# ax-le/nn-fac

Measured on NVIDIA B200. Metric: NMF outer iters/sec (HALS & MU beta=1) at 65536x8192 r=64, higher is better.
Workload: dtype f32

## Files before the change

### nn-fac_b200/csrc/tc_fused.cu

```cuda
#include "tc_plan.cuh"

#include <string.h>

namespace {
using namespace tcplan;

constexpr int NSP = 4;
constexpr int CW = 64 / NSP;
constexpr int NCHK = CW / 8;
constexpr int NWT = 4 * NSP;
constexpr int FUSED_THREADS = 128 + 32 * NWT;
static_assert(CW == 16, "the transform below moves 16 columns per tcgen05.ld / 8 words per tcgen05.st");
constexpr uint32_t X_BYTES = TILE_ROWS * BK * sizeof(bf16);
constexpr int MODE_RES = 0, MODE_MU = 1;
#ifndef FUSED_PREFETCH
#define FUSED_PREFETCH 0
#endif
#ifndef FUSED_PACKED
#define FUSED_PACKED 1
#endif
#ifndef FUSED_DEFER_COST
#define FUSED_DEFER_COST 1
#endif
constexpr int DRAIN = 2;

template <int RK>
struct Cfg {
  static constexpr int KR = RK / 64;
  static constexpr uint32_t FK_BYTES = (uint32_t)KR * 64 * BK * sizeof(bf16);
  static constexpr uint32_t STAGE_BYTES = 2 * X_BYTES + 2 * FK_BYTES;
  static constexpr int FSTAGES = RK == 64 ? 4 : 3;
  static constexpr int ND1 = RK == 64 ? 3 : 2;
  static constexpr uint32_t A1_BYTES = RK == 64 ? 2 * X_BYTES : 0;
  static constexpr int CWD = RK / NSP;
  static constexpr size_t SMEM = A1_BYTES + (size_t)FSTAGES * STAGE_BYTES + 512;
};

struct FusedParams {
  int r_pad, splits, stages_per_unit, num_units, drain, want_cost, tiles, split_major;
  int64_t ld_partial;
  float* partial;
  double* cost_part;
  const bf16 *a1h, *a1l;
  int64_t R;
  float* push[NNFAC_MAX_PEERS];
  int64_t push_chunk;
  int push_src;
};

__device__ __forceinline__ float rcp_approx(float x) {
  float y;
  asm("rcp.approx.ftz.f32 %0, %1;" : "=f"(y) : "f"(x));
  return y;
}
__device__ __forceinline__ float lg2_approx(float x) {
  float y;
  asm("lg2.approx.ftz.f32 %0, %1;" : "=f"(y) : "f"(x));
  return y;
}
__device__ __forceinline__ float bf_lo(uint32_t w) { return __uint_as_float(w << 16); }
__device__ __forceinline__ float bf_hi(uint32_t w) { return __uint_as_float(w & 0xffff0000u); }

template <int MODE, bool COST, bool XF32, int RK>
__global__ void __launch_bounds__(FUSED_THREADS, 1)
tc_fused_kernel(const __grid_constant__ CUtensorMap map_xh, const __grid_constant__ CUtensorMap map_xl,
                const __grid_constant__ CUtensorMap map_fkh, const __grid_constant__ CUtensorMap map_fkl,
                const __grid_constant__ CUtensorMap map_a1h, const __grid_constant__ CUtensorMap map_a1l,
                const FusedParams p) {
  using C = Cfg<RK>;
  static_assert(RK == 64 || (MODE == MODE_RES && !XF32), "rank 65..128: residual + cross-product pass only");
  constexpr int FSTAGES = C::FSTAGES, ND1 = C::ND1, CWD = C::CWD;
  constexpr uint32_t FK_BYTES = C::FK_BYTES, STAGE_BYTES = C::STAGE_BYTES, A1_BYTES = C::A1_BYTES;
  extern __shared__ __align__(1024) uint8_t smem[];
  uint8_t* a1 = smem;
  uint8_t* ring = smem + A1_BYTES;
  uint64_t* bars = reinterpret_cast<uint64_t*>(ring + (size_t)FSTAGES * STAGE_BYTES);
  uint64_t* full = bars;
  uint64_t* empty = bars + 4;
  uint64_t* a1_full = bars + 9;
  uint64_t* a1_empty = bars + 10;
  uint64_t* d1_full = bars + 11;
  uint64_t* d1_empty = bars + 14;
  uint64_t* d2_full = bars + 17;
  uint64_t* d2_empty = bars + 19;
  uint64_t* a1t_ready = bars + 21;
  uint64_t* a1t_free = bars + 22;
  uint64_t* q_ready = bars + 23;
  uint64_t* q_free = bars + 25;
  uint32_t* tmem_slot = reinterpret_cast<uint32_t*>(bars + 27);
  double* cost_sh = reinterpret_cast<double*>(bars + 28);

  const int warp = threadIdx.x >> 5, lane = threadIdx.x & 31;

  if (warp == 0 && lane == 0) {
    tc::prefetch_tmap(&map_xh); tc::prefetch_tmap(&map_xl);
    tc::prefetch_tmap(&map_fkh); tc::prefetch_tmap(&map_fkl);
    if (RK == 64) { tc::prefetch_tmap(&map_a1h); tc::prefetch_tmap(&map_a1l); }
  }
  if (warp == 1 && lane == 0) {
    for (int s = 0; s < FSTAGES; ++s) { tc::mbar_init(&full[s], 1); tc::mbar_init(&empty[s], NWT + 1); }
    tc::mbar_init(a1_full, 1); tc::mbar_init(a1_empty, NWT);
    tc::mbar_init(a1t_ready, NWT); tc::mbar_init(a1t_free, 1);
    for (int b = 0; b < 2; ++b) { tc::mbar_init(&q_ready[b], NWT); tc::mbar_init(&q_free[b], 1); }
    for (int b = 0; b < ND1; ++b) { tc::mbar_init(&d1_full[b], 1); tc::mbar_init(&d1_empty[b], NWT); }
    for (int b = 0; b < 2; ++b) { tc::mbar_init(&d2_full[b], 1); tc::mbar_init(&d2_empty[b], NWT); }
    tc::fence_barrier_init();
  }
  if (warp == 2) tc::tmem_alloc(tmem_slot, 512);
  tc::tcgen05_fence_before();
  __syncthreads();
  tc::tcgen05_fence_after();
  const uint32_t tmem_base = *tmem_slot;
  const uint32_t D1 = tmem_base, D2 = tmem_base + 64 * ND1, A1T = D2 + 2 * RK, QT = A1T + RK;
  const int S = p.stages_per_unit;

  if (warp == 0 && lane == 0) {
    int stage = 0; uint32_t phase = 0, a1_phase = 0;
    for (int u = blockIdx.x; u < p.num_units; u += gridDim.x) {
      const int tile = p.split_major ? u % p.tiles : u / p.splits, split = p.split_major ? u / p.tiles : u % p.splits;
      const int row0 = tile * TILE_ROWS, k0 = split * S * BK;
      if (RK == 64) {
        tc::mbar_wait(a1_empty, a1_phase ^ 1);
        a1_phase ^= 1;
        tc::mbar_arrive_expect_tx(a1_full, A1_BYTES);
        tc::tma_load_2d_hint(a1, &map_a1h, a1_full, 0, row0, tc::kEvictLast);
        tc::tma_load_2d_hint(a1 + X_BYTES, &map_a1l, a1_full, 0, row0, tc::kEvictLast);
      }
      for (int ks = 0; ks < S; ++ks) {
        tc::mbar_wait(&empty[stage], phase ^ 1);
        uint8_t* st = ring + (size_t)stage * STAGE_BYTES;
        tc::mbar_arrive_expect_tx(&full[stage], STAGE_BYTES);
        const int c = k0 + ks * BK;
        tc::tma_load_2d_hint(st, &map_xh, &full[stage], c, row0, tc::kEvictFirst);
        tc::tma_load_2d_hint(st + X_BYTES, XF32 ? &map_xh : &map_xl, &full[stage], XF32 ? c + 32 : c, row0, tc::kEvictFirst);
#pragma unroll
        for (int kr = 0; kr < C::KR; ++kr) {
          tc::tma_load_2d_hint(st + 2 * X_BYTES + kr * 8192, &map_fkh, &full[stage], kr * 64, c, tc::kEvictLast);
          tc::tma_load_2d_hint(st + 2 * X_BYTES + FK_BYTES + kr * 8192, &map_fkl, &full[stage], kr * 64, c, tc::kEvictLast);
        }
        if (++stage == FSTAGES) { stage = 0; phase ^= 1; }
      }
    }
  } else if (warp == 1) {
    const uint32_t idesc1 = tc::umma_idesc_bf16(TILE_ROWS, 64);
    const int ksteps = p.r_pad / UMMA_K;
    int st1 = 0; uint32_t ph1 = 0;
    int b1 = 0; uint32_t b1_phase = 0;
    uint32_t a1_phase = 0;
    for (int u = blockIdx.x; u < p.num_units; u += gridDim.x) {
      tc::mbar_wait(a1t_ready, a1_phase);
      a1_phase ^= 1;
      for (int i = 0; i < S; ++i) {
        tc::mbar_wait(&full[st1], ph1);
        tc::mbar_wait(&d1_empty[b1], b1_phase ^ 1);
        tc::tcgen05_fence_after();
        if (tc::elect_one()) {
          const uint32_t sb = tc::smem_u32(ring + (size_t)st1 * STAGE_BYTES);
          const uint64_t fkh = tc::umma_desc_k_sw128(sb + 2 * X_BYTES), fkl = tc::umma_desc_k_sw128(sb + 2 * X_BYTES + FK_BYTES);
          const uint32_t d = D1 + (uint32_t)b1 * 64;
#pragma unroll
          for (int k = 0; k < RK / UMMA_K; ++k) {
            if (k < ksteps) {
              const uint64_t bo = (uint64_t)((k >> 2) * (8192 >> 4) + (k & 3) * 2);
              tc::umma_bf16_ts(d, A1T + 8 * k, fkh + bo, idesc1, k != 0);
              tc::umma_bf16_ts(d, A1T + RK / 2 + 8 * k, fkh + bo, idesc1, true);
              tc::umma_bf16_ts(d, A1T + 8 * k, fkl + bo, idesc1, true);
            }
          }
          tc::umma_commit(&d1_full[b1]);
          if (i == S - 1) tc::umma_commit(a1t_free);
        }
        __syncwarp();
        if (++b1 == ND1) { b1 = 0; b1_phase ^= 1; }
        if (++st1 == FSTAGES) { st1 = 0; ph1 ^= 1; }
      }
    }
  } else if (warp == 3) {
    const uint32_t idesc2 = tc::umma_idesc_bf16(TILE_ROWS, p.r_pad) | (1u << 16);
    int qb = 0; uint32_t qb_phase = 0;
    int st2 = 0; uint32_t ph2 = 0;
    int b2 = 0; uint32_t b2_phase = 0;
    for (int u = blockIdx.x; u < p.num_units; u += gridDim.x) {
      for (int j = 0; j < S; ++j) {
        const bool chain_start = (j % DRAIN) == 0;
        const bool chain_end = ((j + 1) % DRAIN) == 0 || j == S - 1;
        tc::mbar_wait(&full[st2], ph2);
        if (MODE == MODE_MU) tc::mbar_wait(&q_ready[qb], qb_phase);
        if (chain_start) tc::mbar_wait(&d2_empty[b2], b2_phase ^ 1);
        tc::tcgen05_fence_after();
        if (tc::elect_one()) {
          const uint32_t sb = tc::smem_u32(ring + (size_t)st2 * STAGE_BYTES);
          const uint64_t xh = tc::umma_desc_k_sw128(sb), xl = tc::umma_desc_k_sw128(sb + X_BYTES);
          const uint64_t fnh = tc::umma_desc_mn_sw128(sb + 2 * X_BYTES);
          const uint64_t fnl = tc::umma_desc_mn_sw128(sb + 2 * X_BYTES + FK_BYTES);
          const uint32_t d = D2 + (uint32_t)b2 * RK;
#pragma unroll
          for (int k = 0; k < BK / UMMA_K; ++k) {
            const uint64_t ko = (uint64_t)(k * 2);
            const uint64_t kb = (uint64_t)(k * 128);
            if (MODE == MODE_MU) {
              const uint32_t qa = QT + (uint32_t)qb * 64 + 8 * k;
              tc::umma_bf16_ts(d, qa, fnh + kb, idesc2, !(chain_start && k == 0));
              tc::umma_bf16_ts(d, qa + 32, fnh + kb, idesc2, true);
              tc::umma_bf16_ts(d, qa, fnl + kb, idesc2, true);
            } else {
              tc::umma_bf16(d, xh + ko, fnh + kb, idesc2, !(chain_start && k == 0));
              tc::umma_bf16(d, xl + ko, fnh + kb, idesc2, true);
              tc::umma_bf16(d, xh + ko, fnl + kb, idesc2, true);
            }
          }
          tc::umma_commit(&empty[st2]);
          if (MODE == MODE_MU) tc::umma_commit(&q_free[qb]);
          if (chain_end) tc::umma_commit(&d2_full[b2]);
        }
        __syncwarp();
        if (MODE == MODE_MU) { if (++qb == 2) { qb = 0; qb_phase ^= 1; } }
        if (chain_end) { if (++b2 == 2) { b2 = 0; b2_phase ^= 1; } }
        if (++st2 == FSTAGES) { st2 = 0; ph2 ^= 1; }
      }
    }
  } else if (warp >= 4) {
    const int q = warp & 3, part = (warp - 4) >> 2;
    const int row = q * 32 + lane;
    const uint32_t lane_base = (uint32_t)(q * 32) << 16;
    int st = 0; uint32_t ph = 0;
    int b1 = 0; uint32_t b1_phase = 0;
    int b2 = 0; uint32_t b2_phase = 0;
    int qb = 0; uint32_t qb_phase = 0;
    uint32_t a1_phase = 0;
    double cost = 0.0, costk = 0.0;
    for (int u = blockIdx.x; u < p.num_units; u += gridDim.x) {
      const int tile = p.split_major ? u % p.tiles : u / p.splits, split = p.split_major ? u / p.tiles : u % p.splits;
      float sum[CWD];
#pragma unroll
      for (int j = 0; j < CWD; ++j) sum[j] = 0.f;
      if (RK == 64) {
        tc::mbar_wait(a1_full, a1_phase);
        tc::mbar_wait(a1t_free, a1_phase ^ 1);
        a1_phase ^= 1;
        tc::tcgen05_fence_after();
#pragma unroll
        for (int pl = 0; pl < 2; ++pl) {
          uint32_t w[4 * NCHK];
#pragma unroll
          for (int cc = 0; cc < NCHK; ++cc) {
            const int chunk = NCHK * part + cc;
            const uint4 v4 = *reinterpret_cast<const uint4*>(a1 + pl * X_BYTES + (uint32_t)row * 128u + (uint32_t)((chunk ^ (row & 7)) << 4));
            w[4 * cc] = v4.x; w[4 * cc + 1] = v4.y; w[4 * cc + 2] = v4.z; w[4 * cc + 3] = v4.w;
          }
          tc::tmem_st8(A1T + lane_base + 32 * pl + (CW / 2) * part, w);
        }
        tc::tmem_st_wait();
        tc::tcgen05_fence_before();
        __syncwarp();
        if (lane == 0) { tc::mbar_arrive(a1t_ready); tc::mbar_arrive(a1_empty); }
      } else {
        const int64_t grow = (int64_t)tile * TILE_ROWS + row;
        uint32_t w[2][16];
#pragma unroll
        for (int pl = 0; pl < 2; ++pl) {
          const uint4* src = reinterpret_cast<const uint4*>((pl ? p.a1l : p.a1h) + grow * RK + part * (RK / 4));
#pragma unroll
          for (int c = 0; c < 4; ++c) {
            const uint4 v4 = grow < p.R ? __ldg(src + c) : make_uint4(0u, 0u, 0u, 0u);
            w[pl][4 * c] = v4.x; w[pl][4 * c + 1] = v4.y; w[pl][4 * c + 2] = v4.z; w[pl][4 * c + 3] = v4.w;
          }
        }
        tc::mbar_wait(a1t_free, a1_phase ^ 1);
        a1_phase ^= 1;
        tc::tcgen05_fence_after();
        tc::tmem_st16(A1T + lane_base + (RK / 8) * part, w[0]);
        tc::tmem_st16(A1T + lane_base + RK / 2 + (RK / 8) * part, w[1]);
        tc::tmem_st_wait();
        tc::tcgen05_fence_before();
        __syncwarp();
        if (lane == 0) tc::mbar_arrive(a1t_ready);
      }
      auto drain_chain = [&]() {
        tc::mbar_wait(&d2_full[b2], b2_phase);
        tc::tcgen05_fence_after();
#pragma unroll
        for (int c0 = 0; c0 < CWD; c0 += 16) {
          if (CWD * part + c0 < p.r_pad) {
            uint32_t v[16];
            tc::tmem_ld16(D2 + (uint32_t)b2 * RK + lane_base + CWD * part + c0, v);
            tc::tmem_ld_wait();
#pragma unroll
            for (int j = 0; j < 16; ++j) sum[c0 + j] += __uint_as_float(v[j]);
          }
        }
        tc::tcgen05_fence_before();
        __syncwarp();
        if (lane == 0) tc::mbar_arrive(&d2_empty[b2]);
        if (++b2 == 2) { b2 = 0; b2_phase ^= 1; }
      };
      int drained = 0;
      float2 acc2 = make_float2(0.f, 0.f), acck2 = make_float2(0.f, 0.f);
      const float2 neg1 = make_float2(-1.f, -1.f), tiny2 = make_float2(1e-30f, 1e-30f);
      uint32_t kn[CW];
      int bf = b1; uint32_t bf_phase = b1_phase;
      auto fetch_d1 = [&]() {
        tc::mbar_wait(&d1_full[bf], bf_phase);
        tc::tcgen05_fence_after();
        tc::tmem_ld16(D1 + (uint32_t)bf * 64 + lane_base + CW * part, kn);
        if (++bf == ND1) { bf = 0; bf_phase ^= 1; }
      };
#if FUSED_PREFETCH
      fetch_d1();
#endif
      for (int i = 0; i < S; ++i) {
#if !FUSED_PREFETCH
        fetch_d1();
#endif
        tc::tmem_ld_wait16(kn);
        uint32_t kk[CW];
#pragma unroll
        for (int j = 0; j < CW; ++j) kk[j] = kn[j];
        tc::tcgen05_fence_before();
        __syncwarp();
        if (lane == 0) tc::mbar_arrive(&d1_empty[b1]);
        if (++b1 == ND1) { b1 = 0; b1_phase ^= 1; }
#if FUSED_PREFETCH
        if (i + 1 < S) fetch_d1();
#endif
        tc::mbar_wait(&full[st], ph);
        uint8_t* xh = ring + (size_t)st * STAGE_BYTES;
        uint8_t* xl = xh + X_BYTES;
        uint32_t qhw[4 * NCHK], qlw[4 * NCHK];
        constexpr bool DEFER = FUSED_DEFER_COST && FUSED_PACKED && MODE == MODE_MU && COST;
        float2 xs[DEFER ? 4 * NCHK : 1], qs[DEFER ? 4 * NCHK : 1];
#pragma unroll
        for (int cc = 0; cc < NCHK; ++cc) {
          float2 xv[4];
          if (XF32) {
            const uint8_t* xb = xh + (size_t)(part >> 1) * X_BYTES + (uint32_t)row * 128u;
#pragma unroll
            for (int h = 0; h < 2; ++h) {
              const int chunk = 4 * (part & 1) + 2 * cc + h;
              const float4 v4 = *reinterpret_cast<const float4*>(xb + ((chunk ^ (row & 7)) << 4));
              xv[2 * h] = make_float2(v4.x, v4.y); xv[2 * h + 1] = make_float2(v4.z, v4.w);
            }
          } else {
            const int chunk = NCHK * part + cc;
            const uint32_t off = (uint32_t)row * 128u + (uint32_t)((chunk ^ (row & 7)) << 4);
            const uint4 h4 = *reinterpret_cast<const uint4*>(xh + off);
            const uint4 l4 = *reinterpret_cast<const uint4*>(xl + off);
            const uint32_t hw[4] = {h4.x, h4.y, h4.z, h4.w}, lw[4] = {l4.x, l4.y, l4.z, l4.w};
#pragma unroll
            for (int w = 0; w < 4; ++w)
#if FUSED_PACKED
              xv[w] = __fadd2_rn(make_float2(bf_lo(hw[w]), bf_hi(hw[w])), make_float2(bf_lo(lw[w]), bf_hi(lw[w])));
#else
              xv[w] = make_float2(bf_lo(hw[w]) + bf_lo(lw[w]), bf_hi(hw[w]) + bf_hi(lw[w]));
#endif
          }
#if FUSED_PACKED
#pragma unroll
          for (int w = 0; w < 4; ++w) {
            const float2 x2 = xv[w];
            const float2 k2 = make_float2(__uint_as_float(kk[cc * 8 + 2 * w]), __uint_as_float(kk[cc * 8 + 2 * w + 1]));
            if (MODE == MODE_RES) {
              const float2 r2 = __ffma2_rn(k2, neg1, x2);
              acc2 = __ffma2_rn(r2, r2, acc2);
            } else {
              const float2 kt = __fadd2_rn(k2, tiny2);
              const float2 q2 = __fmul2_rn(x2, make_float2(rcp_approx(kt.x), rcp_approx(kt.y)));
              if (COST) {
                if (DEFER) {
                  xs[DEFER ? 4 * cc + w : 0] = x2; qs[DEFER ? 4 * cc + w : 0] = q2;
                } else {
                  const float2 qt = __fadd2_rn(q2, tiny2);
                  acc2 = __ffma2_rn(x2, make_float2(lg2_approx(qt.x), lg2_approx(qt.y)), acc2);
                }
                acck2 = __fadd2_rn(acck2, k2);
              }
              const __nv_bfloat162 hq = __floats2bfloat162_rn(q2.x, q2.y);
              const uint32_t hqw = *reinterpret_cast<const uint32_t*>(&hq);
              const float2 rem = __ffma2_rn(make_float2(bf_lo(hqw), bf_hi(hqw)), neg1, q2);
              const __nv_bfloat162 lq = __floats2bfloat162_rn(rem.x, rem.y);
              qhw[4 * cc + w] = hqw;
              qlw[4 * cc + w] = *reinterpret_cast<const uint32_t*>(&lq);
            }
          }
#else
#pragma unroll
          for (int w = 0; w < 4; ++w) {
            const float x0 = xv[w].x, x1 = xv[w].y;
            const float k0 = __uint_as_float(kk[cc * 8 + 2 * w]), k1 = __uint_as_float(kk[cc * 8 + 2 * w + 1]);
            if (MODE == MODE_RES) {
              const float r0 = x0 - k0, r1 = x1 - k1;
              acc2.x = fmaf(r0, r0, acc2.x);
              acc2.y = fmaf(r1, r1, acc2.y);
            } else {
              const float i0 = rcp_approx(fmaxf(k0, 1e-30f)), i1 = rcp_approx(fmaxf(k1, 1e-30f));
              const float q0 = x0 * i0, q1 = x1 * i1;
              if (COST) {
                acc2.x = fmaf(x0, lg2_approx(fmaxf(q0, 1e-30f)), acc2.x);
                acc2.y = fmaf(x1, lg2_approx(fmaxf(q1, 1e-30f)), acc2.y);
                acck2.x += k0; acck2.y += k1;
              }
              const __nv_bfloat162 hq = __floats2bfloat162_rn(q0, q1);
              const uint32_t hqw = *reinterpret_cast<const uint32_t*>(&hq);
              const __nv_bfloat162 lq = __floats2bfloat162_rn(q0 - bf_lo(hqw), q1 - bf_hi(hqw));
              qhw[4 * cc + w] = hqw;
              qlw[4 * cc + w] = *reinterpret_cast<const uint32_t*>(&lq);
            }
          }
#endif
        }
        auto flush_cost = [&]() {
          if (COST && ((i & 7) == 7 || i == S - 1)) {
            cost += (double)(acc2.x + acc2.y);
            acc2 = make_float2(0.f, 0.f);
            if (MODE == MODE_MU) { costk += (double)(acck2.x + acck2.y); acck2 = make_float2(0.f, 0.f); }
          }
        };
        if (!DEFER) flush_cost();
        __syncwarp();
        if (lane == 0) tc::mbar_arrive(&empty[st]);
        if (++st == FSTAGES) { st = 0; ph ^= 1; }
        if (MODE == MODE_MU) {
          tc::mbar_wait(&q_free[qb], qb_phase ^ 1);
          tc::tcgen05_fence_after();
          const uint32_t qa = QT + (uint32_t)qb * 64 + lane_base + (CW / 2) * part;
          tc::tmem_st8(qa, qhw);
          tc::tmem_st8(qa + 32, qlw);
          tc::tmem_st_wait();
          tc::tcgen05_fence_before();
          __syncwarp();
          if (lane == 0) tc::mbar_arrive(&q_ready[qb]);
          if (++qb == 2) { qb = 0; qb_phase ^= 1; }
          if (DEFER) {
#pragma unroll
            for (int e = 0; e < 4 * NCHK; ++e) {
              const float2 qt = __fadd2_rn(qs[DEFER ? e : 0], tiny2);
              acc2 = __ffma2_rn(xs[DEFER ? e : 0], make_float2(lg2_approx(qt.x), lg2_approx(qt.y)), acc2);
            }
            flush_cost();
          }
        }
        if (i >= 3 && (i & 1)) { drain_chain(); ++drained; }
      }
      for (; drained < (S + DRAIN - 1) / DRAIN; ++drained) drain_chain();
      if (p.push_chunk > 0) {
        const int64_t row0 = (int64_t)tile * TILE_ROWS;
        const int q = (int)(row0 / p.push_chunk);
        float* out = p.push[q] + (((int64_t)p.push_src * p.splits + split) * p.r_pad + CWD * part) * p.push_chunk + (row0 - q * p.push_chunk) + row;
#pragma unroll
        for (int j = 0; j < CWD; ++j)
          if (CWD * part + j < p.r_pad) out[(int64_t)j * p.push_chunk] = sum[j];
      } else {
        float* out = p.partial + ((int64_t)split * p.r_pad + CWD * part) * p.ld_partial + (int64_t)tile * TILE_ROWS + row;
#pragma unroll
        for (int j = 0; j < CWD; ++j)
          if (CWD * part + j < p.r_pad) out[(int64_t)j * p.ld_partial] = sum[j];
      }
    }
    if (COST) {
      cost = warp_sum(cost);
      if (MODE == MODE_MU) costk = warp_sum(costk);
      if (lane == 0) { cost_sh[warp - 4] = cost; cost_sh[NWT + warp - 4] = costk; }
      asm volatile("bar.sync 1, %0;" ::"n"(32 * NWT) : "memory");
      if (warp == 4 && lane == 0) {
        double t = 0.0, tk = 0.0;
        for (int w = 0; w < NWT; ++w) { t += cost_sh[w]; tk += cost_sh[NWT + w]; }
        p.cost_part[blockIdx.x] = t;
        p.cost_part[512 + blockIdx.x] = tk;
      }
    }
  }
  tc::tcgen05_fence_before();
  __syncthreads();
  if (warp == 2) tc::tmem_dealloc(tmem_base, 512);
}

struct PeerG {
  const float* p[NNFAC_MAX_PEERS];
  const unsigned long long* flags;
  int world;
  unsigned long long seq;
};

template <bool APPLY, int RK, bool PULL>
__global__ void __launch_bounds__(256) factor_finish_kernel(const float* __restrict__ partial, int splits, int r, int r_pad, int64_t R,
                                                            int64_t ldp, const float* __restrict__ F_in, int64_t ld_in,
                                                            int64_t in_chunk, int64_t in_slab, const PeerG G,
                                                            const float* __restrict__ den, float floor_value, float* __restrict__ F_out,
                                                            int64_t ld_out, bf16* __restrict__ fh, bf16* __restrict__ fl, int64_t ld_plane,
                                                            bf16* __restrict__ rowh, bf16* __restrict__ rowl) {
  __shared__ float tile[RK][33];
  const int tx = threadIdx.x & 31, ty = threadIdx.x >> 5;
  if (PULL && G.flags != nullptr) {
    if ((int)threadIdx.x < G.world) {
      const unsigned long long* f = G.flags + NNFAC_MAX_PEERS + threadIdx.x;
      unsigned long long v, spins = 0;
      do {
        asm volatile("ld.acquire.sys.global.u64 %0, [%1];" : "=l"(v) : "l"(f) : "memory");
        if (++spins > (1ull << 27)) __trap();
      } while (v < G.seq);
    }
    __syncthreads();
  }
  const int64_t c0 = (int64_t)blockIdx.x * 32, c = c0 + tx;
  const int64_t cin = in_chunk > 0 ? (c / in_chunk) * in_slab + (c % in_chunk) : c;
  float pulled[PULL ? RK / 8 : 1];
  if (PULL) {
    const float* src = c < R ? G.p[c / in_chunk] + (c % in_chunk) : nullptr;
#pragma unroll
    for (int i = 0; i < RK / 8; ++i) {
      const int k = ty + 8 * i;
      pulled[i] = (k < r && c < R) ? __ldcv(src + (int64_t)k * ld_in) : 0.f;
    }
  }
#pragma unroll
  for (int k = ty; k < RK; k += 8) {
    float f = 0.f;
    if (k < r && c < R) {
      f = PULL ? pulled[PULL ? (k - ty) / 8 : 0] : F_in[(int64_t)k * ld_in + cin];
      if (APPLY) {
        float num = 0.f;
        int sp = 0;
        for (; sp + 8 <= splits; sp += 8) {
          float t[8];
#pragma unroll
          for (int u = 0; u < 8; ++u) t[u] = partial[((int64_t)(sp + u) * r_pad + k) * ldp + c];
#pragma unroll
          for (int u = 0; u < 8; ++u) num += t[u];
        }
        for (; sp < splits; ++sp) num += partial[((int64_t)sp * r_pad + k) * ldp + c];
        const float v = f * (num / den[k]);
        f = v > floor_value ? v : floor_value;
        if (v != v) f = v;
      }
      if (F_out) F_out[(int64_t)k * ld_out + c] = f;
      bf16 h, l;
      tc::split_bf16(f, h, l);
      fh[(int64_t)k * ld_plane + c] = h;
      fl[(int64_t)k * ld_plane + c] = l;
    }
    tile[k][tx] = f;
  }
  if (rowh == nullptr) return;
  __syncthreads();
  for (int i = ty; i < 32; i += 8) {
    const int64_t cc = c0 + i;
    if (cc < R) {
#pragma unroll
      for (int h2 = 0; h2 < RK / 32; ++h2) {
        const int k = tx + 32 * h2;
        bf16 h, l;
        tc::split_bf16(tile[k][i], h, l);
        rowh[cc * RK + k] = h;
        rowl[cc * RK + k] = l;
      }
    }
  }
}

__global__ void sum_cost_parts_kernel(const double* part, int n, double* out) {
  if (threadIdx.x == 0) {
    double s = 0.0;
    for (int i = 0; i < n; ++i) s += part[i];
    out[0] = s;
  }
}

__global__ void kl_cost_finish_kernel(const double* part, int n, const double* sums, double* out) {
  if (threadIdx.x == 0) {
    double s = 0.0, sk = 0.0;
    for (int i = 0; i < n; ++i) { s += part[i]; sk += part[512 + i]; }
    constexpr double a0 = 6.05e-8, a1 = -4.0e-8;
    s = (1.0 - a1) * s - a0 * sums[0];
    out[0] = 0.6931471805599453 * s - sums[0] + sk;
  }
}

__global__ void __launch_bounds__(256) planes_to_f32_kernel(const bf16* __restrict__ hi, const bf16* __restrict__ lo, int64_t count,
                                                            float* __restrict__ out) {
  const int64_t stride = (int64_t)gridDim.x * blockDim.x * 2;
  for (int64_t i = ((int64_t)blockIdx.x * blockDim.x + threadIdx.x) * 2; i < count; i += stride) {
    const uint32_t h = *reinterpret_cast<const uint32_t*>(hi + i), l = *reinterpret_cast<const uint32_t*>(lo + i);
    *reinterpret_cast<float2*>(out + i) = make_float2(bf_lo(h) + bf_lo(l), bf_hi(h) + bf_hi(l));
  }
}

}

static int finish_factor(nnfac_nmf_plan* p, int which, bool apply, const float* F_in, int64_t ld_in, int64_t in_chunk, int64_t in_slab,
                         const float* den, float floor_value, float* F_out, int64_t ld_out, cudaStream_t st, const PeerG* pulled = nullptr) {
  const int64_t len = which == 0 ? p->m : p->n;
  Side* cs = &p->side[which == 0 ? 1 : 0];
  Side* ps = &p->side[which];
  const unsigned grid = (unsigned)ceil_div64(len, 32);
  bf16* rh = p->fused_ok ? p->rowp_h[which] : nullptr;
  bf16* rl = p->fused_ok ? p->rowp_l[which] : nullptr;
  PeerG none;
  memset(&none, 0, sizeof(none));
#define NNFAC_FINISH(RKV)                                                                                                          \
  do {                                                                                                                             \
    if (pulled)                                                                                                                    \
      factor_finish_kernel<false, RKV, true><<<grid, 256, 0, st>>>(nullptr, 0, p->r, p->r_pad, len, 0, nullptr, ld_in, in_chunk,  \
          in_slab, *pulled, nullptr, 0.f, F_out, ld_out, cs->fh, cs->fl, cs->ld, rh, rl);                                          \
    else if (apply)                                                                                                                \
      factor_finish_kernel<true, RKV, false><<<grid, 256, 0, st>>>(p->partial, ps->cp.splits, p->r, p->r_pad, len,                \
          ps->cp.ld_partial, F_in, ld_in, in_chunk, in_slab, none, den, floor_value, F_out, ld_out, cs->fh, cs->fl, cs->ld, rh,    \
          rl);                                                                                                                     \
    else                                                                                                                           \
      factor_finish_kernel<false, RKV, false><<<grid, 256, 0, st>>>(nullptr, 0, p->r, p->r_pad, len, 0, F_in, ld_in, in_chunk,    \
          in_slab, none, nullptr, 0.f, F_out, ld_out, cs->fh, cs->fl, cs->ld, rh, rl);                                             \
  } while (0)
  if (p->rk == 64) NNFAC_FINISH(64); else NNFAC_FINISH(128);
#undef NNFAC_FINISH
  NNFAC_LAUNCH_CHECK(p->ctx);
  return NNFAC_OK;
}

extern "C" {

int nnfac_nmf_plan_f32_bytes(const nnfac_nmf_plan* p, size_t* bytes) {
  NNFAC_ARG(p && bytes, "nnfac_nmf_plan_f32_bytes: NULL argument");
  size_t tot = 0;
  for (int i = 0; i < 2; ++i) tot += (((size_t)p->side[i].R * p->side[i].ld * sizeof(float)) + 255) & ~(size_t)255;
  *bytes = tot;
  return NNFAC_OK;
}

int nnfac_nmf_plan_enable_f32(nnfac_nmf_plan* p, void* workspace, size_t workspace_bytes, void* stream) {
  NNFAC_ARG(p && workspace && (((uintptr_t)workspace) & 255) == 0, "nnfac_nmf_plan_enable_f32: bad argument");
  size_t need = 0;
  nnfac_nmf_plan_f32_bytes(p, &need);
  NNFAC_ARG(workspace_bytes >= need, "nnfac_nmf_plan_enable_f32: workspace of %zu bytes needed, got %zu", need, workspace_bytes);
  NNFAC_ARG(p->sides == 3, "nnfac_nmf_plan_enable_f32: needs a two-sided plan");
  if (!p->fused_ok || p->rk != 64) { nnfac_set_error("nnfac_nmf_plan_enable_f32: rank %d > 64 is not covered by the beta = 1 fused pass", p->r); return NNFAC_ERR_UNSUPPORTED; }
  cudaStream_t st = (cudaStream_t)stream;
  uint8_t* base = (uint8_t*)workspace;
  for (int i = 0; i < 2; ++i) {
    Side* s = &p->side[i];
    p->xf[i] = (float*)base;
    const int64_t count = s->R * s->ld;
    base += (((size_t)count * sizeof(float)) + 255) & ~(size_t)255;
    planes_to_f32_kernel<<<p->ctx->sm_count * 16, 256, 0, st>>>(s->xh, s->xl, count, p->xf[i]);
    NNFAC_LAUNCH_CHECK(p->ctx);
    const int rc = make_map_f32(&p->map_xf[i], p->xf[i], s->R, s->C, s->ld);
    if (rc) return rc;
  }
  p->xf_ready = 1;
  return NNFAC_OK;
}

int nnfac_nmf_plan_set_factor(nnfac_nmf_plan* p, int which, const float* Ft, int64_t ld, void* stream) {
  NNFAC_ARG(p && Ft && (which == 0 || which == 1), "nnfac_nmf_plan_set_factor: bad argument");
  NNFAC_ARG(!p->base, "nnfac_nmf_plan_set_factor: not available on a view plan");
  const int64_t len = which == 0 ? p->m : p->n;
  NNFAC_ARG(ld >= len, "nnfac_nmf_plan_set_factor: leading dimension too small");
  return finish_factor(p, which, false, Ft, ld, 0, 0, nullptr, 0.f, nullptr, 0, (cudaStream_t)stream);
}

int nnfac_nmf_plan_set_factor_gathered(nnfac_nmf_plan* p, int which, const float* G, int64_t chunk, float* Ft_out, int64_t ld_out,
                                       void* stream) {
  NNFAC_ARG(p && G && Ft_out && chunk > 0 && (which == 0 || which == 1), "nnfac_nmf_plan_set_factor_gathered: bad argument");
  const int64_t len = which == 0 ? p->m : p->n;
  NNFAC_ARG(ld_out >= len, "nnfac_nmf_plan_set_factor_gathered: leading dimension too small");
  return finish_factor(p, which, false, G, chunk, chunk, (int64_t)p->r * chunk, nullptr, 0.f, Ft_out, ld_out, (cudaStream_t)stream);
}

const float* nnfac_xchg_peer_send(const nnfac_xchg* x, int q);
int nnfac_xchg_world(const nnfac_xchg* x);
void nnfac_xchg_wait_args(const nnfac_xchg* x, int phase, const unsigned long long** flags, int* world, unsigned long long* seq);
int nnfac_nmf_plan_set_factor_pulled(nnfac_nmf_plan* p, int which, const nnfac_xchg* x, int64_t chunk, int64_t pitch, float* Ft_out,
                                     int64_t ld_out, void* stream) {
  NNFAC_ARG(p && x && Ft_out && chunk > 0 && pitch >= chunk && (which == 0 || which == 1), "nnfac_nmf_plan_set_factor_pulled: bad argument");
  NNFAC_ARG(!p->base, "nnfac_nmf_plan_set_factor_pulled: not available on a view plan");
  const int64_t len = which == 0 ? p->m : p->n;
  const int world = nnfac_xchg_world(x);
  NNFAC_ARG(ld_out >= len && (int64_t)world * chunk >= len, "nnfac_nmf_plan_set_factor_pulled: %d slices of %lld columns do not cover %lld",
            world, (long long)chunk, (long long)len);
  PeerG g;
  for (int q = 0; q < NNFAC_MAX_PEERS; ++q) g.p[q] = nnfac_xchg_peer_send(x, q);
  nnfac_xchg_wait_args(x, 1, &g.flags, &g.world, &g.seq);
  return finish_factor(p, which, false, nullptr, pitch, chunk, 0, nullptr, 0.f, Ft_out, ld_out, (cudaStream_t)stream, &g);
}

int nnfac_nmf_plan_hals_solve(nnfac_nmf_plan* p, int which, const float* UtM, int64_t ld_utm, const float* UtU, int64_t ld_utu,
                              const float* F_in, int64_t ld_in, float* F_out, int64_t ld_out, int maxiter, double delta,
                              double sparsity, double* result, void* stream) {
  NNFAC_ARG(p && UtU && F_in && F_out && result && (which == 0 || which == 1), "nnfac_nmf_plan_hals_solve: bad argument");
  NNFAC_ARG(!p->base, "nnfac_nmf_plan_hals_solve: not available on a view plan");
  const int64_t len = which == 0 ? p->m : p->n;
  NNFAC_ARG((!UtM || ld_utm >= len) && ld_in >= len && ld_out >= len && ld_utu >= p->r, "nnfac_nmf_plan_hals_solve: leading dimension too small");
  int nsplit = 1;
  int64_t split_stride = 0;
  if (!UtM) {
    const CrossParams& cp = p->side[which].cp;
    UtM = p->partial; ld_utm = cp.ld_partial; nsplit = cp.splits; split_stride = (int64_t)p->r_pad * cp.ld_partial;
  }
  Side* cs = &p->side[which == 0 ? 1 : 0];
  nnfac_sweep_planes pl;
  pl.fh = cs->fh; pl.fl = cs->fl; pl.ld_plane = cs->ld; pl.r_pad = p->r_pad;
  pl.rowh = p->fused_ok ? p->rowp_h[which] : nullptr;
  pl.rowl = p->fused_ok ? p->rowp_l[which] : nullptr;
  pl.row_pitch = p->rk;
  return nnfac_tc_sweep_run(p->ctx, UtM, ld_utm, UtU, ld_utu, F_in, ld_in, F_out, ld_out, p->r, len, maxiter, delta, sparsity,
                            result, &pl, (cudaStream_t)stream, nsplit, split_stride);
}

void* nnfac_xchg_peer_stage(const nnfac_xchg* x, int q);
int nnfac_xchg_rank(const nnfac_xchg* x);
int64_t nnfac_xchg_stage_floats(const nnfac_xchg* x);
int nnfac_nmf_plan_set_push(nnfac_nmf_plan* p, const nnfac_xchg* x, int64_t inbox_off, int64_t chunk, int* slabs, int64_t* slab_stride) {
  NNFAC_ARG(p, "nnfac_nmf_plan_set_push: NULL plan");
  if (!x) { p->push_chunk = 0; return NNFAC_OK; }
  NNFAC_ARG(!p->base && p->fused_ok, "nnfac_nmf_plan_set_push: needs a plan with the fused pass");
  const int world = nnfac_xchg_world(x);
  const int splits = p->side[0].cp.splits;
  NNFAC_ARG(chunk > 0 && chunk % TILE_ROWS == 0 && (int64_t)world * chunk >= p->m && inbox_off >= 0,
            "nnfac_nmf_plan_set_push: %d slices of %lld rows (multiple of 128) must cover %lld", world, (long long)chunk, (long long)p->m);
  NNFAC_ARG(inbox_off + (int64_t)world * splits * p->r_pad * chunk <= nnfac_xchg_stage_floats(x),
            "nnfac_nmf_plan_set_push: the stage buffer is too small for %d x %d slabs of %d x %lld", world, splits, p->r_pad, (long long)chunk);
  for (int q = 0; q < world; ++q) p->push[q] = (float*)nnfac_xchg_peer_stage(x, q) + inbox_off;
  p->push_chunk = chunk; p->push_src = nnfac_xchg_rank(x); p->push_world = world;
  if (slabs) *slabs = world * splits;
  if (slab_stride) *slab_stride = (int64_t)p->r_pad * chunk;
  return NNFAC_OK;
}

int nnfac_reduce_slabs_f32(nnfac_ctx* ctx, const float* slabs, int64_t ld, int nslabs, int r, int r_pad, int64_t n, float* out,
                           int64_t ld_out, void* stream) {
  NNFAC_ARG(ctx && slabs && out && nslabs >= 1 && r >= 1 && r_pad >= r && n >= 1 && ld >= n && ld_out >= n, "nnfac_reduce_slabs_f32: bad argument");
  nnfac_reduce_partials(slabs, nslabs, r, r_pad, n, ld, out, ld_out, ctx->sm_count, (cudaStream_t)stream);
  NNFAC_LAUNCH_CHECK(ctx);
  return NNFAC_OK;
}

int nnfac_nmf_plan_reduce(nnfac_nmf_plan* p, int side, float* out, int64_t ld_out, void* stream) {
  NNFAC_ARG(p && out && (side == 0 || side == 1), "nnfac_nmf_plan_reduce: bad argument");
  Side* s = &p->side[side];
  NNFAC_ARG(ld_out >= s->R, "nnfac_nmf_plan_reduce: leading dimension too small");
  nnfac_reduce_partials(p->partial, s->cp.splits, p->r, p->r_pad, s->R, s->cp.ld_partial, out, ld_out, p->ctx->sm_count, (cudaStream_t)stream);
  NNFAC_LAUNCH_CHECK(p->ctx);
  return NNFAC_OK;
}

int nnfac_nmf_plan_reduce_chunked(nnfac_nmf_plan* p, int side, float* out, int64_t chunk, int slabs, const float* tail, int64_t ld_tail,
                                  int tail_cols, void* stream) {
  NNFAC_ARG(p && out && (side == 0 || side == 1) && chunk > 0 && slabs > 0 && tail_cols >= 0 && (tail || tail_cols == 0),
            "nnfac_nmf_plan_reduce_chunked: bad argument");
  Side* s = &p->side[side];
  NNFAC_ARG((int64_t)slabs * chunk >= s->R, "nnfac_nmf_plan_reduce_chunked: %d slabs of %lld columns do not cover %lld", slabs,
            (long long)chunk, (long long)s->R);
  nnfac_reduce_partials_chunked(p->partial, s->cp.splits, p->r, p->r_pad, s->R, s->cp.ld_partial, out, chunk, slabs, tail, ld_tail,
                                tail_cols, p->ctx->sm_count, (cudaStream_t)stream);
  NNFAC_LAUNCH_CHECK(p->ctx);
  return NNFAC_OK;
}

int nnfac_nmf_plan_mu_finish(nnfac_nmf_plan* p, int which, const float* F_in, int64_t ld_in, const float* den, double floor_value,
                             float* F_out, int64_t ld_out, void* stream) {
  NNFAC_ARG(p && F_in && den && F_out && (which == 0 || which == 1), "nnfac_nmf_plan_mu_finish: bad argument");
  const int64_t len = which == 0 ? p->m : p->n;
  NNFAC_ARG(ld_in >= len && ld_out >= len, "nnfac_nmf_plan_mu_finish: leading dimension too small");
  if (!p->fused_ok) { nnfac_set_error("nnfac_nmf_plan_mu_finish: rank %d > 128 is not covered by the fused pass", p->r); return NNFAC_ERR_UNSUPPORTED; }
  return finish_factor(p, which, true, F_in, ld_in, 0, 0, den, (float)floor_value, F_out, ld_out, (cudaStream_t)stream);
}

int nnfac_nmf_plan_fused(nnfac_nmf_plan* p, int side, int mode, int want_cost, float* out, int64_t ld_out, double* cost_out,
                         void* stream) {
  NNFAC_ARG(p && (side == 0 || side == 1) && (mode == 0 || mode == 1), "nnfac_nmf_plan_fused: bad argument");
  NNFAC_ARG((p->sides >> side) & 1, "nnfac_nmf_plan_fused: this plan keeps no planes of side %d", side);
  if (!p->fused_ok) { nnfac_set_error("nnfac_nmf_plan_fused: not covered by the fused pass (rank %d > 128, or a view plan)", p->r); return NNFAC_ERR_UNSUPPORTED; }
  if (mode == 1 && p->rk != 64) { nnfac_set_error("nnfac_nmf_plan_fused: the beta = 1 pass covers rank <= 64 (rank %d)", p->r); return NNFAC_ERR_UNSUPPORTED; }
  Side* s = &p->side[side];
  NNFAC_ARG(!out || ld_out >= s->R, "nnfac_nmf_plan_fused: leading dimension too small");
  cudaStream_t st = (cudaStream_t)stream;
  FusedParams fp;
  fp.r_pad = p->r_pad; fp.splits = s->cp.splits; fp.stages_per_unit = s->cp.stages_per_unit; fp.num_units = s->cp.num_units;
  fp.drain = DRAIN; fp.want_cost = (mode == 0 || want_cost) ? 1 : 0;
  fp.tiles = s->cp.tiles; fp.split_major = s->cp.split_major;
  fp.ld_partial = s->cp.ld_partial; fp.partial = p->partial; fp.cost_part = p->cost_part;
  fp.a1h = p->rowp_h[side]; fp.a1l = p->rowp_l[side]; fp.R = s->R;
  fp.push_chunk = 0; fp.push_src = 0;
  for (int q = 0; q < NNFAC_MAX_PEERS; ++q) fp.push[q] = nullptr;
  if (side == 0 && !out && p->push_chunk > 0) {
    fp.push_chunk = p->push_chunk; fp.push_src = p->push_src;
    for (int q = 0; q < p->push_world; ++q) fp.push[q] = p->push[q];
  }
  const int other = 1 - side;
#define NNFAC_LAUNCH_FUSED(M, C, XF, RKV, MAPH, MAPL)                                                                             \
  do {                                                                                                                        \
    const size_t smem = Cfg<RKV>::SMEM;                                                                                       \
    NNFAC_CUDA(cudaFuncSetAttribute(tc_fused_kernel<M, C, XF, RKV>, cudaFuncAttributeMaxDynamicSharedMemorySize, (int)smem)); \
    tc_fused_kernel<M, C, XF, RKV><<<s->grid, FUSED_THREADS, smem, st>>>(MAPH, MAPL, p->map_row_b_h[other],                  \
        p->map_row_b_l[other], p->map_row_a_h[side], p->map_row_a_l[side], fp);                                               \
  } while (0)
  if (mode == 0 && p->rk == 128) NNFAC_LAUNCH_FUSED(MODE_RES, true, false, 128, s->map_xh, s->map_xl);
  else if (mode == 0) NNFAC_LAUNCH_FUSED(MODE_RES, true, false, 64, s->map_xh, s->map_xl);
  else if (p->xf_ready) {
    if (fp.want_cost) NNFAC_LAUNCH_FUSED(MODE_MU, true, true, 64, p->map_xf[side], p->map_xf[side]);
    else NNFAC_LAUNCH_FUSED(MODE_MU, false, true, 64, p->map_xf[side], p->map_xf[side]);
  } else {
    if (fp.want_cost) NNFAC_LAUNCH_FUSED(MODE_MU, true, false, 64, s->map_xh, s->map_xl);
    else NNFAC_LAUNCH_FUSED(MODE_MU, false, false, 64, s->map_xh, s->map_xl);
  }
#undef NNFAC_LAUNCH_FUSED
  NNFAC_LAUNCH_CHECK(p->ctx);
  if (out) {
    nnfac_reduce_partials(p->partial, fp.splits, p->r, p->r_pad, s->R, fp.ld_partial, out, ld_out, p->ctx->sm_count, st);
    NNFAC_LAUNCH_CHECK(p->ctx);
  }
  if (cost_out && fp.want_cost) {
    if (mode == 0)
      sum_cost_parts_kernel<<<1, 32, 0, st>>>(p->cost_part, s->grid, cost_out);
    else
      kl_cost_finish_kernel<<<1, 32, 0, st>>>(p->cost_part, s->grid, p->sums, cost_out);
    NNFAC_LAUNCH_CHECK(p->ctx);
  }
  return NNFAC_OK;
}

}
```

Measured before the change: 776.5.

## Split fused kernel smem ring into separate X and factor rings with independent producers

Splits the single shared-memory stage ring (X tile plus factor slices) into two rings with their own full/empty barriers and a second TMA producer warp, so X and factor loads progress independently. The factor ring is released by the MMA warps via commits, while the X ring is released by the transform warps. In residual mode the X ring is released early, right after the values are read into registers. This lets factor stages be recycled without waiting for the slower elementwise consumers. The cost is more barriers, extra registers for X values held across the loop, and configurable ring depths that must fit in shared memory.

```diff
diff --git a/nn-fac_b200/csrc/tc_fused.cu b/nn-fac_b200/csrc/tc_fused.cu
--- a/nn-fac_b200/csrc/tc_fused.cu
+++ b/nn-fac_b200/csrc/tc_fused.cu
@@ -19,21 +19,43 @@
 #ifndef FUSED_PACKED
 #define FUSED_PACKED 1
 #endif
+#ifndef FUSED_X_FIRST
+#define FUSED_X_FIRST 0
+#endif
+#ifndef FUSED_MU_LATE_X
+#define FUSED_MU_LATE_X 1
+#endif
 #ifndef FUSED_DEFER_COST
 #define FUSED_DEFER_COST 1
 #endif
 constexpr int DRAIN = 2;
+#ifndef FUSED_XST64
+#define FUSED_XST64 4
+#endif
+#ifndef FUSED_SST64
+#define FUSED_SST64 4
+#endif
+#ifndef FUSED_XST128
+#define FUSED_XST128 3
+#endif
+#ifndef FUSED_SST128
+#define FUSED_SST128 3
+#endif
 
 template <int RK>
 struct Cfg {
   static constexpr int KR = RK / 64;
   static constexpr uint32_t FK_BYTES = (uint32_t)KR * 64 * BK * sizeof(bf16);
-  static constexpr uint32_t STAGE_BYTES = 2 * X_BYTES + 2 * FK_BYTES;
-  static constexpr int FSTAGES = RK == 64 ? 4 : 3;
+  static constexpr uint32_t XS_BYTES = 2 * X_BYTES;
+  static constexpr uint32_t SS_BYTES = 2 * FK_BYTES;
+  static constexpr int XST = RK == 64 ? FUSED_XST64 : FUSED_XST128;
+  static constexpr int SST = RK == 64 ? FUSED_SST64 : FUSED_SST128;
   static constexpr int ND1 = RK == 64 ? 3 : 2;
   static constexpr uint32_t A1_BYTES = RK == 64 ? 2 * X_BYTES : 0;
   static constexpr int CWD = RK / NSP;
-  static constexpr size_t SMEM = A1_BYTES + (size_t)FSTAGES * STAGE_BYTES + 512;
+  static constexpr int NBAR = 2 * XST + 2 * SST + 2 * ND1 + 10;
+  static constexpr size_t SMEM = A1_BYTES + (size_t)XST * XS_BYTES + (size_t)SST * SS_BYTES + 8 * (NBAR + 1 + 2 * NWT);
+  static_assert(SMEM <= 227 * 1024, "ring depths exceed the shared memory of a block");
 };
 
 struct FusedParams {
@@ -69,26 +91,30 @@
                 const FusedParams p) {
   using C = Cfg<RK>;
   static_assert(RK == 64 || (MODE == MODE_RES && !XF32), "rank 65..128: residual + cross-product pass only");
-  constexpr int FSTAGES = C::FSTAGES, ND1 = C::ND1, CWD = C::CWD;
-  constexpr uint32_t FK_BYTES = C::FK_BYTES, STAGE_BYTES = C::STAGE_BYTES, A1_BYTES = C::A1_BYTES;
+  constexpr int XST = C::XST, SST = C::SST, ND1 = C::ND1, CWD = C::CWD;
+  constexpr uint32_t FK_BYTES = C::FK_BYTES, XS_BYTES = C::XS_BYTES, SS_BYTES = C::SS_BYTES, A1_BYTES = C::A1_BYTES;
   extern __shared__ __align__(1024) uint8_t smem[];
   uint8_t* a1 = smem;
-  uint8_t* ring = smem + A1_BYTES;
-  uint64_t* bars = reinterpret_cast<uint64_t*>(ring + (size_t)FSTAGES * STAGE_BYTES);
-  uint64_t* full = bars;
-  uint64_t* empty = bars + 4;
-  uint64_t* a1_full = bars + 9;
-  uint64_t* a1_empty = bars + 10;
-  uint64_t* d1_full = bars + 11;
-  uint64_t* d1_empty = bars + 14;
-  uint64_t* d2_full = bars + 17;
-  uint64_t* d2_empty = bars + 19;
-  uint64_t* a1t_ready = bars + 21;
-  uint64_t* a1t_free = bars + 22;
-  uint64_t* q_ready = bars + 23;
-  uint64_t* q_free = bars + 25;
-  uint32_t* tmem_slot = reinterpret_cast<uint32_t*>(bars + 27);
-  double* cost_sh = reinterpret_cast<double*>(bars + 28);
+  uint8_t* xring = smem + A1_BYTES;
+  uint8_t* sring = xring + (size_t)XST * XS_BYTES;
+  uint64_t* bars = reinterpret_cast<uint64_t*>(sring + (size_t)SST * SS_BYTES);
+  uint64_t* x_full = bars;
+  uint64_t* x_empty = x_full + XST;
+  uint64_t* s_full = x_empty + XST;
+  uint64_t* s_empty = s_full + SST;
+  uint64_t* a1_full = s_empty + SST;
+  uint64_t* a1_empty = a1_full + 1;
+  uint64_t* d1_full = a1_empty + 1;
+  uint64_t* d1_empty = d1_full + ND1;
+  uint64_t* d2_full = d1_empty + ND1;
+  uint64_t* d2_empty = d2_full + 2;
+  uint64_t* a1t_ready = d2_empty + 2;
+  uint64_t* a1t_free = a1t_ready + 1;
+  uint64_t* q_ready = a1t_free + 1;
+  uint64_t* q_free = q_ready + 2;
+  static_assert(2 * XST + 2 * SST + 2 * ND1 + 10 == C::NBAR, "barrier block");
+  uint32_t* tmem_slot = reinterpret_cast<uint32_t*>(bars + C::NBAR);
+  double* cost_sh = reinterpret_cast<double*>(bars + C::NBAR + 1);
 
   const int warp = threadIdx.x >> 5, lane = threadIdx.x & 31;
 
@@ -98,7 +124,8 @@
     if (RK == 64) { tc::prefetch_tmap(&map_a1h); tc::prefetch_tmap(&map_a1l); }
   }
   if (warp == 1 && lane == 0) {
-    for (int s = 0; s < FSTAGES; ++s) { tc::mbar_init(&full[s], 1); tc::mbar_init(&empty[s], NWT + 1); }
+    for (int s = 0; s < XST; ++s) { tc::mbar_init(&x_full[s], 1); tc::mbar_init(&x_empty[s], MODE == MODE_MU ? NWT : NWT + 1); }
+    for (int s = 0; s < SST; ++s) { tc::mbar_init(&s_full[s], 1); tc::mbar_init(&s_empty[s], 2); }
     tc::mbar_init(a1_full, 1); tc::mbar_init(a1_empty, NWT);
     tc::mbar_init(a1t_ready, NWT); tc::mbar_init(a1t_free, 1);
     for (int b = 0; b < 2; ++b) { tc::mbar_init(&q_ready[b], NWT); tc::mbar_init(&q_free[b], 1); }
@@ -115,6 +142,21 @@
   const int S = p.stages_per_unit;
 
   if (warp == 0 && lane == 0) {
+    int stage = 0; uint32_t phase = 0;
+    for (int u = blockIdx.x; u < p.num_units; u += gridDim.x) {
+      const int tile = p.split_major ? u % p.tiles : u / p.splits, split = p.split_major ? u / p.tiles : u % p.splits;
+      const int row0 = tile * TILE_ROWS, k0 = split * S * BK;
+      for (int ks = 0; ks < S; ++ks) {
+        tc::mbar_wait(&x_empty[stage], phase ^ 1);
+        uint8_t* st = xring + (size_t)stage * XS_BYTES;
+        tc::mbar_arrive_expect_tx(&x_full[stage], XS_BYTES);
+        const int c = k0 + ks * BK;
+        tc::tma_load_2d_hint(st, &map_xh, &x_full[stage], c, row0, tc::kEvictFirst);
+        tc::tma_load_2d_hint(st + X_BYTES, XF32 ? &map_xh : &map_xl, &x_full[stage], XF32 ? c + 32 : c, row0, tc::kEvictFirst);
+        if (++stage == XST) { stage = 0; phase ^= 1; }
+      }
+    }
+  } else if (warp == 2 && lane == 0) {
     int stage = 0; uint32_t phase = 0, a1_phase = 0;
     for (int u = blockIdx.x; u < p.num_units; u += gridDim.x) {
       const int tile = p.split_major ? u % p.tiles : u / p.splits, split = p.split_major ? u / p.tiles : u % p.splits;
@@ -127,18 +169,16 @@
         tc::tma_load_2d_hint(a1 + X_BYTES, &map_a1l, a1_full, 0, row0, tc::kEvictLast);
       }
       for (int ks = 0; ks < S; ++ks) {
-        tc::mbar_wait(&empty[stage], phase ^ 1);
-        uint8_t* st = ring + (size_t)stage * STAGE_BYTES;
-        tc::mbar_arrive_expect_tx(&full[stage], STAGE_BYTES);
+        tc::mbar_wait(&s_empty[stage], phase ^ 1);
+        uint8_t* st = sring + (size_t)stage * SS_BYTES;
+        tc::mbar_arrive_expect_tx(&s_full[stage], SS_BYTES);
         const int c = k0 + ks * BK;
-        tc::tma_load_2d_hint(st, &map_xh, &full[stage], c, row0, tc::kEvictFirst);
-        tc::tma_load_2d_hint(st + X_BYTES, XF32 ? &map_xh : &map_xl, &full[stage], XF32 ? c + 32 : c, row0, tc::kEvictFirst);
 #pragma unroll
         for (int kr = 0; kr < C::KR; ++kr) {
-          tc::tma_load_2d_hint(st + 2 * X_BYTES + kr * 8192, &map_fkh, &full[stage], kr * 64, c, tc::kEvictLast);
-          tc::tma_load_2d_hint(st + 2 * X_BYTES + FK_BYTES + kr * 8192, &map_fkl, &full[stage], kr * 64, c, tc::kEvictLast);
-        }
-        if (++stage == FSTAGES) { stage = 0; phase ^= 1; }
+          tc::tma_load_2d_hint(st + kr * 8192, &map_fkh, &s_full[stage], kr * 64, c, tc::kEvictLast);
+          tc::tma_load_2d_hint(st + FK_BYTES + kr * 8192, &map_fkl, &s_full[stage], kr * 64, c, tc::kEvictLast);
+        }
+        if (++stage == SST) { stage = 0; phase ^= 1; }
       }
     }
   } else if (warp == 1) {
@@ -151,12 +191,12 @@
       tc::mbar_wait(a1t_ready, a1_phase);
       a1_phase ^= 1;
       for (int i = 0; i < S; ++i) {
-        tc::mbar_wait(&full[st1], ph1);
+        tc::mbar_wait(&s_full[st1], ph1);
         tc::mbar_wait(&d1_empty[b1], b1_phase ^ 1);
         tc::tcgen05_fence_after();
         if (tc::elect_one()) {
-          const uint32_t sb = tc::smem_u32(ring + (size_t)st1 * STAGE_BYTES);
-          const uint64_t fkh = tc::umma_desc_k_sw128(sb + 2 * X_BYTES), fkl = tc::umma_desc_k_sw128(sb + 2 * X_BYTES + FK_BYTES);
+          const uint32_t sb = tc::smem_u32(sring + (size_t)st1 * SS_BYTES);
+          const uint64_t fkh = tc::umma_desc_k_sw128(sb), fkl = tc::umma_desc_k_sw128(sb + FK_BYTES);
           const uint32_t d = D1 + (uint32_t)b1 * 64;
 #pragma unroll
           for (int k = 0; k < RK / UMMA_K; ++k) {
@@ -168,31 +208,35 @@
             }
           }
           tc::umma_commit(&d1_full[b1]);
+          tc::umma_commit(&s_empty[st1]);
           if (i == S - 1) tc::umma_commit(a1t_free);
         }
         __syncwarp();
         if (++b1 == ND1) { b1 = 0; b1_phase ^= 1; }
-        if (++st1 == FSTAGES) { st1 = 0; ph1 ^= 1; }
+        if (++st1 == SST) { st1 = 0; ph1 ^= 1; }
       }
     }
   } else if (warp == 3) {
     const uint32_t idesc2 = tc::umma_idesc_bf16(TILE_ROWS, p.r_pad) | (1u << 16);
     int qb = 0; uint32_t qb_phase = 0;
     int st2 = 0; uint32_t ph2 = 0;
+    int xs2 = 0; uint32_t xph2 = 0;
     int b2 = 0; uint32_t b2_phase = 0;
     for (int u = blockIdx.x; u < p.num_units; u += gridDim.x) {
       for (int j = 0; j < S; ++j) {
         const bool chain_start = (j % DRAIN) == 0;
         const bool chain_end = ((j + 1) % DRAIN) == 0 || j == S - 1;
-        tc::mbar_wait(&full[st2], ph2);
+        tc::mbar_wait(&s_full[st2], ph2);
         if (MODE == MODE_MU) tc::mbar_wait(&q_ready[qb], qb_phase);
+        else tc::mbar_wait(&x_full[xs2], xph2);
         if (chain_start) tc::mbar_wait(&d2_empty[b2], b2_phase ^ 1);
         tc::tcgen05_fence_after();
         if (tc::elect_one()) {
-          const uint32_t sb = tc::smem_u32(ring + (size_t)st2 * STAGE_BYTES);
-          const uint64_t xh = tc::umma_desc_k_sw128(sb), xl = tc::umma_desc_k_sw128(sb + X_BYTES);
-          const uint64_t fnh = tc::umma_desc_mn_sw128(sb + 2 * X_BYTES);
-          const uint64_t fnl = tc::umma_desc_mn_sw128(sb + 2 * X_BYTES + FK_BYTES);
+          const uint32_t xb = tc::smem_u32(xring + (size_t)xs2 * XS_BYTES);
+          const uint64_t xh = tc::umma_desc_k_sw128(xb), xl = tc::umma_desc_k_sw128(xb + X_BYTES);
+          const uint32_t sb = tc::smem_u32(sring + (size_t)st2 * SS_BYTES);
+          const uint64_t fnh = tc::umma_desc_mn_sw128(sb);
+          const uint64_t fnl = tc::umma_desc_mn_sw128(sb + FK_BYTES);
           const uint32_t d = D2 + (uint32_t)b2 * RK;
 #pragma unroll
           for (int k = 0; k < BK / UMMA_K; ++k) {
@@ -209,14 +253,16 @@
               tc::umma_bf16(d, xh + ko, fnl + kb, idesc2, true);
             }
           }
-          tc::umma_commit(&empty[st2]);
+          tc::umma_commit(&s_empty[st2]);
           if (MODE == MODE_MU) tc::umma_commit(&q_free[qb]);
+          else tc::umma_commit(&x_empty[xs2]);
           if (chain_end) tc::umma_commit(&d2_full[b2]);
         }
         __syncwarp();
         if (MODE == MODE_MU) { if (++qb == 2) { qb = 0; qb_phase ^= 1; } }
+        else { if (++xs2 == XST) { xs2 = 0; xph2 ^= 1; } }
         if (chain_end) { if (++b2 == 2) { b2 = 0; b2_phase ^= 1; } }
-        if (++st2 == FSTAGES) { st2 = 0; ph2 ^= 1; }
+        if (++st2 == SST) { st2 = 0; ph2 ^= 1; }
       }
     }
   } else if (warp >= 4) {
@@ -309,7 +355,51 @@
       fetch_d1();
 #endif
       for (int i = 0; i < S; ++i) {
-#if !FUSED_PREFETCH
+#if !FUSED_PREFETCH && !FUSED_X_FIRST
+        fetch_d1();
+#endif
+        tc::mbar_wait(&x_full[st], ph);
+        float2 xv[NCHK][4];
+        {
+          const uint8_t* xh = xring + (size_t)st * XS_BYTES;
+          const uint8_t* xl = xh + X_BYTES;
+#pragma unroll
+          for (int cc = 0; cc < NCHK; ++cc) {
+            if (XF32) {
+              const uint8_t* xb = xh + (size_t)(part >> 1) * X_BYTES + (uint32_t)row * 128u;
+#pragma unroll
+              for (int h = 0; h < 2; ++h) {
+                const int chunk = 4 * (part & 1) + 2 * cc + h;
+                const float4 v4 = *reinterpret_cast<const float4*>(xb + ((chunk ^ (row & 7)) << 4));
+                xv[cc][2 * h] = make_float2(v4.x, v4.y); xv[cc][2 * h + 1] = make_float2(v4.z, v4.w);
+              }
+            } else {
+              const int chunk = NCHK * part + cc;
+              const uint32_t off = (uint32_t)row * 128u + (uint32_t)((chunk ^ (row & 7)) << 4);
+              const uint4 h4 = *reinterpret_cast<const uint4*>(xh + off);
+              const uint4 l4 = *reinterpret_cast<const uint4*>(xl + off);
+              const uint32_t hw[4] = {h4.x, h4.y, h4.z, h4.w}, lw[4] = {l4.x, l4.y, l4.z, l4.w};
+#pragma unroll
+              for (int w = 0; w < 4; ++w)
+#if FUSED_PACKED
+                xv[cc][w] = __fadd2_rn(make_float2(bf_lo(hw[w]), bf_hi(hw[w])), make_float2(bf_lo(lw[w]), bf_hi(lw[w])));
+#else
+                xv[cc][w] = make_float2(bf_lo(hw[w]) + bf_lo(lw[w]), bf_hi(hw[w]) + bf_hi(lw[w]));
+#endif
+            }
+          }
+        }
+        constexpr bool EARLY_X = MODE == MODE_RES || !FUSED_MU_LATE_X;
+        auto release_x = [&]() {
+          __syncwarp();
+          if (lane == 0) tc::mbar_arrive(&x_empty[st]);
+          if (++st == XST) { st = 0; ph ^= 1; }
+        };
+        if (EARLY_X) {
+          tc::fence_proxy_async_smem();
+          release_x();
+        }
+#if !FUSED_PREFETCH && FUSED_X_FIRST
         fetch_d1();
 #endif
         tc::tmem_ld_wait16(kn);
@@ -323,41 +413,15 @@
 #if FUSED_PREFETCH
         if (i + 1 < S) fetch_d1();
 #endif
-        tc::mbar_wait(&full[st], ph);
-        uint8_t* xh = ring + (size_t)st * STAGE_BYTES;
-        uint8_t* xl = xh + X_BYTES;
         uint32_t qhw[4 * NCHK], qlw[4 * NCHK];
         constexpr bool DEFER = FUSED_DEFER_COST && FUSED_PACKED && MODE == MODE_MU && COST;
         float2 xs[DEFER ? 4 * NCHK : 1], qs[DEFER ? 4 * NCHK : 1];
 #pragma unroll
         for (int cc = 0; cc < NCHK; ++cc) {
-          float2 xv[4];
-          if (XF32) {
-            const uint8_t* xb = xh + (size_t)(part >> 1) * X_BYTES + (uint32_t)row * 128u;
-#pragma unroll
-            for (int h = 0; h < 2; ++h) {
-              const int chunk = 4 * (part & 1) + 2 * cc + h;
-              const float4 v4 = *reinterpret_cast<const float4*>(xb + ((chunk ^ (row & 7)) << 4));
-              xv[2 * h] = make_float2(v4.x, v4.y); xv[2 * h + 1] = make_float2(v4.z, v4.w);
-            }
-          } else {
-            const int chunk = NCHK * part + cc;
-            const uint32_t off = (uint32_t)row * 128u + (uint32_t)((chunk ^ (row & 7)) << 4);
-            const uint4 h4 = *reinterpret_cast<const uint4*>(xh + off);
-            const uint4 l4 = *reinterpret_cast<const uint4*>(xl + off);
-            const uint32_t hw[4] = {h4.x, h4.y, h4.z, h4.w}, lw[4] = {l4.x, l4.y, l4.z, l4.w};
-#pragma unroll
-            for (int w = 0; w < 4; ++w)
 #if FUSED_PACKED
-              xv[w] = __fadd2_rn(make_float2(bf_lo(hw[w]), bf_hi(hw[w])), make_float2(bf_lo(lw[w]), bf_hi(lw[w])));
-#else
-              xv[w] = make_float2(bf_lo(hw[w]) + bf_lo(lw[w]), bf_hi(hw[w]) + bf_hi(lw[w]));
-#endif
-          }
-#if FUSED_PACKED
 #pragma unroll
           for (int w = 0; w < 4; ++w) {
-            const float2 x2 = xv[w];
+            const float2 x2 = xv[cc][w];
             const float2 k2 = make_float2(__uint_as_float(kk[cc * 8 + 2 * w]), __uint_as_float(kk[cc * 8 + 2 * w + 1]));
             if (MODE == MODE_RES) {
               const float2 r2 = __ffma2_rn(k2, neg1, x2);
@@ -385,7 +449,7 @@
 #else
 #pragma unroll
           for (int w = 0; w < 4; ++w) {
-            const float x0 = xv[w].x, x1 = xv[w].y;
+            const float x0 = xv[cc][w].x, x1 = xv[cc][w].y;
             const float k0 = __uint_as_float(kk[cc * 8 + 2 * w]), k1 = __uint_as_float(kk[cc * 8 + 2 * w + 1]);
             if (MODE == MODE_RES) {
               const float r0 = x0 - k0, r1 = x1 - k1;
@@ -416,9 +480,7 @@
           }
         };
         if (!DEFER) flush_cost();
-        __syncwarp();
-        if (lane == 0) tc::mbar_arrive(&empty[st]);
-        if (++st == FSTAGES) { st = 0; ph ^= 1; }
+        if (!EARLY_X) release_x();
         if (MODE == MODE_MU) {
           tc::mbar_wait(&q_free[qb], qb_phase ^ 1);
           tc::tcgen05_fence_after();
@@ -471,7 +533,10 @@
   }
   tc::tcgen05_fence_before();
   __syncthreads();
-  if (warp == 2) tc::tmem_dealloc(tmem_base, 512);
+  if (warp == 2) {
+    __syncwarp();
+    tc::tmem_dealloc(tmem_base, 512);
+  }
 }
 
 struct PeerG {
```

Result: no change. 782.0, median of 6 (+0.7%).
